# factoryofthesun/distraytracer

Hardware: NVIDIA B200
Metric: samples_per_s_1080p_64spp (higher is better)
Workload: dtype f64

## Files before the change

### distraytracer_b200/csrc/drt_api.cu

```cuda
#include <cuda_runtime.h>

#include <algorithm>
#include <cmath>
#include <cstdio>
#include <cstdlib>
#include <cstring>
#include <string>
#include <vector>

#include "../../include/drt.h"
#include "drt_box.cuh"
#include "drt_launch.h"
#include "drt_bvh_order.h"
#include "drt_mesh.h"
#include "drt_skeleton.h"

using namespace drt;

namespace {

thread_local std::string g_err;
int fail(int code, const std::string& m) { g_err = m; return code; }

#define CK(call)                                                                                   \
// ... 787 lines not shown
int finishRender(drt_scene* s, drt_counters* counters, const Counts& hc, int overflowed) {
  if (overflowed) {
    CK(cudaMemsetAsync(s->overflow, 0, sizeof(int), s->stream));
    CK(cudaStreamSynchronize(s->stream));
    return fail(DRT_ERR_UNSUPPORTED, "a CTA ray pool overflowed (brdf_samples * max_depth beyond the sized bound)");
  }
  if (counters) {
    float ms = 0; CK(cudaEventElapsedTime(&ms, s->ev0, s->ev1));
    counters->kernel_ms = ms;
    if (counters->collect) {
      counters->samples = hc.samples; counters->rays = hc.rays; counters->shadow_rays = hc.shadow_rays;
      counters->shade_evals = hc.shade_evals; counters->noise_evals = hc.noise_evals; counters->node_tests = hc.node_tests;
      for (int i = 0; i < DRT_PRIM_TYPE_COUNT; i++) counters->prim_tests[i] = 0;
      counters->prim_tests[DRT_PRIM_SPHERE] = hc.geom_tests[G_SPHERE];
      counters->prim_tests[DRT_PRIM_CYLINDER] = hc.geom_tests[G_CYL];
      counters->prim_tests[DRT_PRIM_TRIANGLE] = hc.geom_tests[G_TRI];
      counters->prim_tests[DRT_PRIM_RECTANGLE] = hc.geom_tests[G_RECT] + hc.geom_tests[G_CHECKER];
      counters->prim_tests[DRT_PRIM_RECTPRISM] = hc.geom_tests[G_BOX];
    }
  }
  return DRT_OK;
}

int readBack(drt_scene* s, drt_counters* counters, bool check_overflow) {
  Counts hc; memset(&hc, 0, sizeof(hc));
  if (counters && counters->collect) CK(cudaMemcpyAsync(&hc, s->counts, sizeof(Counts), cudaMemcpyDeviceToHost, s->stream));
  int overflowed = 0;
  if (check_overflow) CK(cudaMemcpyAsync(&overflowed, s->overflow, sizeof(int), cudaMemcpyDeviceToHost, s->stream));
  CK(cudaStreamSynchronize(s->stream));
  return finishRender(s, counters, hc, overflowed);
}

int renderCommon(const drt_scene* cs, const drt_settings* st, const drt_tile* tile, float* out_f32, uint8_t* out_u8,
                 drt_counters* counters, bool copy_back) {
  drt_scene* s = const_cast<drt_scene*>(cs);
  int pool_cap = 0;
  CameraD cam;
  int rc = planRender(s, st, tile, pool_cap, cam);
  if (rc) return rc;
  if (tile->device != s->device) return fail(DRT_ERR_INVALID, "tile.device differs from the scene's device");
  CK(cudaSetDevice(s->device));
  const bool want_f32 = out_f32 != nullptr;
  rc = launchFor(s, st, cam, tile, pool_cap, want_f32, counters);
  if (rc) return rc;
  const size_t n_out = (size_t)tile->width * tile->height * 3;
  if (copy_back) {
    if (out_u8) CK(cudaMemcpyAsync(out_u8, s->out_u8, n_out, cudaMemcpyDeviceToHost, s->stream));
    if (out_f32) CK(cudaMemcpyAsync(out_f32, s->out_f32, n_out * sizeof(float), cudaMemcpyDeviceToHost, s->stream));
  }
  return readBack(s, counters, !st->cloud_only);
}

// ... 375 lines not shown
void drt_abi_sizes(int32_t* out6) {
  out6[0] = (int32_t)sizeof(drt_prim); out6[1] = (int32_t)sizeof(drt_light); out6[2] = (int32_t)sizeof(drt_scene_desc);
  out6[3] = (int32_t)sizeof(drt_settings); out6[4] = (int32_t)sizeof(drt_tile); out6[5] = (int32_t)sizeof(drt_counters);
}

int drt_debug_candidate_order(const drt_prim* prims, int32_t n_prims, int32_t* out, int32_t cap) {
  if (!prims || n_prims < 1 || !out) return 0;
  int n = 0;
  for (int i : referenceBVH(prims, n_prims).order) { if (n < cap) out[n] = i; n++; }
  return n;
}

float drt_debug_rng(uint32_t seed, uint32_t pixel, uint32_t sample, uint32_t child, uint32_t dim) {
  uint32_t pk = rng_key_pixel(seed, pixel);
  uint32_t sk = rng_key_sample(pk, sample);
  return rng_u01(rng_key_child(sk, child), dim);
}

int drt_debug_shuffle_j(uint32_t seed, uint32_t pixel, int32_t i) { return rng_shuffle_j(rng_key_pixel(seed, pixel), i); }
int drt_debug_lens_index(uint32_t seed, uint32_t pixel, int32_t sample, int32_t n_lens) {
  return lensIndexScan(rng_key_pixel(seed, pixel), sample, n_lens);
}

}
```

### distraytracer_b200/csrc/drt_device.cuh

```cuda
#pragma once
#include <cuda_runtime.h>
#include <stdint.h>
#include <float.h>
#include <math.h>
#include <utility>

#include "drt_rng.cuh"

#define DRT_PI 3.14159265358979323846
#define DRT_NODE_STACK 64

namespace drt {

template <typename R> struct Vec { R x, y, z; };

template <typename R> __host__ __device__ inline Vec<R> mk(R x, R y, R z) { Vec<R> v; v.x = x; v.y = y; v.z = z; return v; }
template <typename R> __host__ __device__ inline Vec<R> operator+(Vec<R> a, Vec<R> b) { return mk<R>(a.x + b.x, a.y + b.y, a.z + b.z); }
template <typename R> __host__ __device__ inline Vec<R> operator-(Vec<R> a, Vec<R> b) { return mk<R>(a.x - b.x, a.y - b.y, a.z - b.z); }
template <typename R> __host__ __device__ inline Vec<R> operator-(Vec<R> a) { return mk<R>(-a.x, -a.y, -a.z); }
template <typename R> __host__ __device__ inline Vec<R> operator*(Vec<R> a, R s) { return mk<R>(a.x * s, a.y * s, a.z * s); }
template <typename R> __host__ __device__ inline Vec<R> operator*(R s, Vec<R> a) { return mk<R>(s * a.x, s * a.y, s * a.z); }
template <typename R> __host__ __device__ inline Vec<R> operator/(Vec<R> a, R s) { return mk<R>(a.x / s, a.y / s, a.z / s); }
template <typename R> __host__ __device__ inline R dot(Vec<R> a, Vec<R> b) { return a.x * b.x + (a.y * b.y + a.z * b.z); }
template <typename R> __host__ __device__ inline R norm(Vec<R> a) { return sqrt(dot(a, a)); }
// ... 84 lines not shown
  R objM[12];
  Vec<R> center, eA, eB, eC, eD; R e_den;
  Vec<R> vel;
  float height; int n_holes;
  HoleD<R> holes[4];
};

template <typename R>
struct alignas(16) MeshTri {
  Vec<R> A, B, C;
  float uv[6];
};

template <typename R>
struct alignas(16) LightD {
  int type, prim_index;
  float radius;
  int use_baxis;
  float color[3];
  float pad_;
  Vec<R> center, baxis, A, B, D;
};

struct Counts {
  unsigned long long samples, rays, shadow_rays, geom_tests[7], shade_evals, noise_evals, node_tests;
};

template <typename R>
struct Params {
  Vec<R> eye, X, Y, Z;
  R mcam[12], new_mcam[12], cloud_mcam[12];
  float t, b, r, l;
  float near_plane, focal_length, aperture;
  int xRes, yRes;
  int n, spp, antialias_samples;
  int brdf_samples, blur_samples, frame_range, max_depth;
  int reflect, nogloss, perlin_cloud, cloud_only;
  int frame, frame_prism, frame_blur, frame_cloud;
  int swept_cull;
  float move_per_frame, accel_t, refr_air, refr_glass, phong;
  uint32_t seed;
  int blur_mode;
  Vec<R> sun;
  float sun_outer[3], sun_inner[3], sun_core[3], bluesky[3], redsky[3];
  float saturation, clouddist, cloudhoff;
  int x0, y0, w, h;
  const Geom<R>* geoms; int n_geoms;
  const float4* gbounds;
// ... 59 lines not shown
```

### distraytracer_b200/csrc/drt_kernels.cuh

```cuda
#pragma once
#include "drt_device.cuh"
#include "drt_launch.h"
#include <cstddef>

#ifndef DRT_FORCE_TREE
#define DRT_FORCE_TREE 0
#endif

namespace drt {


template <typename R>
struct alignas(16) Task {
  Vec<R> org, dir;
  float k;
  uint32_t path;
  float dt;
  unsigned char depth;
  unsigned char bits;
  unsigned short slot;
};
#define TASK_CHAIN 1
#define TASK_ROOT 2
static_assert(sizeof(Task<double>) == 64 && sizeof(Task<float>) == 48, "ray records are whole 16-byte words");
// ... 329 lines not shown
struct HitRec {
  float t;
  int geom;
  int inside;
  int checker_sel;
};

template <typename R, int F>
__device__ inline bool geomIntersect(const Params<R>& P, const Geom<R>& g, int gi, const int type, const Moved<R>& mv,
                                     const Vec<R>& ray, const Vec<R>& start, float& t_hit, int& inside, int& sel) {
  bool ok = false;
  inside = 0; sel = 0;
    if ((F & FT_BOX) && type == G_BOX) {
      return boxIntersect<R>(P.prims[g.owner], shiftPoint<R, F>(mv, 0, g.vel, g.p0), shiftPoint<R, F>(mv, 0, g.vel, g.p1), ray, start, t_hit, inside, sel);
    } else if (type == G_RECT || type == G_CHECKER) {
      Vec<R> A = shiftPoint<R, F>(mv, g.flags, g.vel, g.p0);
      if (type == G_CHECKER) {
        if (dot(g.p1, ray) == R(0)) return false;
      }
      float c1, c2;
      ok = rectHit<R>(A, g.p1, g.p2, g.p3, g.len1, g.len2, g.eps, ray, start, t_hit, c1, c2);
      if (ok && type == G_CHECKER) {
        if (g.flags & GF_HAS_HOLE) {
          const Geom<R>& hgeo = P.geoms[gi + 1];
          float th, d1, d2;
          if (rectHit<R>(hgeo.p0, hgeo.p1, hgeo.p2, hgeo.p3, hgeo.len1, hgeo.len2, hgeo.eps, ray, start, th, d1, d2))
            ok = false;
        }
        if (ok) {
          int i = (int)(c1 / g.f2);
          int j = (int)(c2 / g.f2);
          int pi = i % 2, pj = j % 2;
          if (pi == 0) { if (pj == 0) sel = 1; if (pj == 1) sel = 2; }
          if (pi == 1) { if (pj == 0) sel = 2; if (pj == 1) sel = 1; }
        }
      }
    } else if (type == G_SPHERE) {
      Vec<R> sc = start - shiftPoint<R, F>(mv, g.flags, g.vel, g.p0);
      float A = (float)dot(ray, ray);
      float B = (float)(R(2) * dot(ray, sc));
      float C = (float)(dot(sc, sc) - (R)((double)g.f0 * (double)g.f0));
      float disc = (float)((double)B * (double)B - (double)(4 * A * C));
      if (disc < 0) return false;
      float sq = sqrtf(disc);
      float t0 = (-B + sq) / (2 * A);
      float t1 = (-B - sq) / (2 * A);
      if (t0 <= 0.001f && t1 <= 0.001f) return false;
// ... 177 lines not shown
    if (ok2 && k2 != kb) stack[sp++] = make_int2(r2, __float_as_int(t2));
    if (ok3 && k3 != kb) stack[sp++] = make_int2(r3, __float_as_int(t3));
    const int bk = kb & 3;
    return bk == 0 ? r0 : bk == 1 ? r1 : bk == 2 ? r2 : r3;
  }
  int nxt = DRT_MESH_DONE;
  if (ok0) nxt = r0;
  if (ok1) { if (nxt != DRT_MESH_DONE) stack[sp++] = make_int2(nxt, 0); nxt = r1; }
  if (ok2) { if (nxt != DRT_MESH_DONE) stack[sp++] = make_int2(nxt, 0); nxt = r2; }
  if (ok3) { if (nxt != DRT_MESH_DONE) stack[sp++] = make_int2(nxt, 0); nxt = r3; }
  return (nxt != DRT_MESH_DONE) ? nxt : bvh4Pop<CLOSEST>(stack, sp, sr.lim);
}

template <typename R, int F, bool COUNT>
__device__ __noinline__ bool gatherReplay(const Params<R>& P, const int leaf, const Vec<R> ray, const Vec<R> start, const Moved<R> mv, Counts& cnt) {
  const Vec<R> inv_ray = mk<R>(R(1) / ray.x, R(1) / ray.y, R(1) / ray.z);
  for (int ni = leaf; ni >= 0; ni = P.nodes[ni].parent) {
    if (COUNT) cnt.node_tests++;
    if (!boxHit<R, F>(P.nodes[ni], ray, inv_ray, start, mv)) return false;
  }
  return true;
}

template <typename R, int F, bool COUNT>
__device__ inline void closestHit(const Params<R>& P, const SlabTab gb, const Moved<R>& mv, const Vec<R>& ray,
                                  const Vec<R>& start, HitRec& h, Counts& cnt) {
  h.t = FLT_MAX; h.geom = -1; h.inside = 0; h.checker_sel = 0;
  if ((!(F & FT_REFBLUR) || mv.val == 0.0f) && !DRT_FORCE_TREE) {
    const float ix = 1.0f / (float)ray.x, iy = 1.0f / (float)ray.y, iz = 1.0f / (float)ray.z;
    const float ox = -(float)start.x * ix, oy = -(float)start.y * iy, oz = -(float)start.z * iz;
    const float serr = 4e-7f * (fabsf(ox) + fabsf(oy) + fabsf(oz));
    const bool cull = !((F & FT_VEL) && mv.velocity_mode) || P.swept_cull;
    const bool smem = !(F & FT_BIG) || P.n_geoms <= DRT_SMEM_GEOMS;
    if ((F & FT_BIG) && cull && P.geom_tree) {
      SlabRay st = slabRay(ix, iy, iz, ox, oy, oz, FLT_MAX);
      int2 stack[DRT_NODE_STACK];
      int sp = 0, cur = 0;
      for (;;) {
        while (cur >= 0) { if (COUNT) cnt.node_tests += 4; cur = bvh4Visit<true>(P.geom_tree, cur, st, stack, sp, P.overflow); }
        if (cur == DRT_MESH_DONE) break;
        const int gi = -cur - 1;
        const Geom<R>& g = P.geoms[gi];
        const int type = g.type;
        if (COUNT) cnt.geom_tests[type]++;
        float t_hit; int inside, sel;
        if (geomIntersect<R, F>(P, g, gi, type, mv, ray, start, t_hit, inside, sel) && (t_hit < h.t || (t_hit == h.t && gi < h.geom)) &&
            (!(F & FT_SPILL) || !(g.flags & GF_SPILL) || ((F & FT_VEL) && mv.velocity_mode) || gatherReplay<R, F, COUNT>(P, g.leaf, ray, start, mv, cnt))) {
          h.t = t_hit; h.geom = gi; h.inside = inside; h.checker_sel = sel;
          st.lim = (t_hit * 1.0001f + 1e-4f) + serr;
        }
        cur = bvh4Pop<true>(stack, sp, st.lim);
      }
      return;
    }
    const SlabRay sr = slabRay(ix, iy, iz, ox, oy, oz, FLT_MAX);
    const int n = P.n_geoms;
    for (int g0 = 0; g0 < n; g0 += 32) {
      const int g1 = min(n, g0 + 32);
      unsigned int mask = !cull ? slabAll(g0, g1) : smem ? slabMask<true>(gb, n, g0, g1, sr) : slabMask<false>(gb, n, g0, g1, sr);
      while (mask) {
        const int gi = g0 + __ffs(mask) - 1;
        mask &= mask - 1;
        const Geom<R>& g = P.geoms[gi];
        const int type = g.type;
        if (type == G_HOLE) continue;
        if (cull && h.t < FLT_MAX && !slabMayHit(g.blo, g.bhi, ox, oy, oz, ix, iy, iz, h.t * 1.0001f + 1e-4f, serr)) continue;
        if (COUNT) cnt.geom_tests[type]++;
        float t_hit; int inside, sel;
        if (geomIntersect<R, F>(P, g, gi, type, mv, ray, start, t_hit, inside, sel) && t_hit < h.t &&
            (!(F & FT_SPILL) || !(g.flags & GF_SPILL) || ((F & FT_VEL) && mv.velocity_mode) || gatherReplay<R, F, COUNT>(P, g.leaf, ray, start, mv, cnt))) {
          h.t = t_hit; h.geom = gi; h.inside = inside; h.checker_sel = sel;
        }
      }
    }
    return;
  }
  int stack[DRT_NODE_STACK];
  int sp = 0;
  stack[sp++] = 0;
  const Vec<R> inv_ray = mk<R>(R(1) / ray.x, R(1) / ray.y, R(1) / ray.z);
  while (sp > 0) {
    const NodeD<R>& nd = P.nodes[stack[--sp]];
    if (COUNT) cnt.node_tests++;
    if (!boxHit<R, F>(nd, ray, inv_ray, start, mv)) continue;
    if (!nd.leaf) { stack[sp++] = nd.left; stack[sp++] = nd.right; continue; }
    const int g_end = nd.first + nd.count;
    for (int gi = nd.first; gi < g_end; gi++) {
      const Geom<R>& g = P.geoms[gi];
      const int type = g.type;
      if (type == G_HOLE) continue;
      if (COUNT) cnt.geom_tests[type]++;
      float t_hit; int inside, sel;
      if (geomIntersect<R, F>(P, g, gi, type, mv, ray, start, t_hit, inside, sel) && t_hit < h.t) {
        h.t = t_hit; h.geom = gi; h.inside = inside; h.checker_sel = sel;
      }
    }
  }
}

template <typename R, int F>
__device__ inline bool geomShadow(const Params<R>& P, const Geom<R>& g, int gi, const int type, const Moved<R>& mv,
                                  const Vec<R>& ray, const Vec<R>& start, const float t_max, float& t_occ, bool& aborted) {
    t_occ = 0.0f;
    if ((F & FT_BOX) && type == G_BOX) {
      return boxShadow<R>(P.prims[g.owner], shiftPoint<R, F>(mv, 0, g.vel, g.p0), shiftPoint<R, F>(mv, 0, g.vel, g.p1), ray, start, t_max, aborted);
    } else if (type == G_RECT || type == G_CHECKER) {
      Vec<R> A = shiftPoint<R, F>(mv, g.flags, g.vel, g.p0);
      float eps = (type == G_CHECKER && !(g.flags & GF_HAS_HOLE)) ? 1e-4f : g.eps;
      float th, c1, c2;
      if (rectHit<R>(A, g.p1, g.p2, g.p3, g.len1, g.len2, eps, ray, start, th, c1, c2) && th < t_max) {
        if (g.flags & GF_HAS_HOLE) {
          const Geom<R>& hgeo = P.geoms[gi + 1];
          float t2, d1, d2;
          if (rectHit<R>(hgeo.p0, hgeo.p1, hgeo.p2, hgeo.p3, hgeo.len1, hgeo.len2, hgeo.eps, ray, start, t2, d1, d2) &&
              t2 < t_max)
            return false;
        }
        t_occ = th;
        return true;
      }
    } else if (type == G_SPHERE) {
      const float eps = 1e-3f;
      Vec<R> sc = start - shiftPoint<R, F>(mv, g.flags, g.vel, g.p0);
      float A = (float)dot(ray, ray);
      float B = (float)(R(2) * dot(ray, sc));
      float C = (float)(dot(sc, sc) - (R)((double)g.f0 * (double)g.f0));
      float disc = (float)((double)B * (double)B - (double)(4 * A * C));
      if (disc < 0) return false;
      float sq = sqrtf(disc);
      float t0 = (-B + sq) / (2 * A);
      float t1 = (-B - sq) / (2 * A);
      if ((t0 <= eps || t0 >= t_max) && (t1 <= eps || t1 >= t_max)) return false;
      t_occ = (t0 > eps && t0 < t_max) ? t0 : t1;
      return true;
    } else if (type == G_CYL) {
// ... 32 lines not shown
      Vec<R> DA0 = cross(A0, r1);
      float v = (float)((double)dot(ray, DA0) * (double)invdet);
      if (v < 0 || u + v > 1) return false;
      float t_final = (float)((double)dot(r2, DA0) * (double)invdet);
      if (t_final > 0.001f && t_final < t_max) { t_occ = t_final; return true; }
    }
  return false;
}

template <typename R, int F, bool COUNT>
__device__ inline bool anyHit(const Params<R>& P, const SlabTab gb, const Moved<R>& mv, const Vec<R>& gather_ray,
                              const Vec<R>& gather_start, const Vec<R>& ray, const Vec<R>& start, float t_max, int skip_owner,
                              Counts& cnt, bool& aborted) {
  if ((!(F & FT_REFBLUR) || mv.val == 0.0f) && !DRT_FORCE_TREE) {
    const float ix = 1.0f / (float)ray.x, iy = 1.0f / (float)ray.y, iz = 1.0f / (float)ray.z;
    const float ox = -(float)start.x * ix, oy = -(float)start.y * iy, oz = -(float)start.z * iz;
    const bool cull = !((F & FT_VEL) && mv.velocity_mode) || P.swept_cull;
    const float gather_lead = t_max * 1e-3f;
    const int n = P.n_geoms;
    const bool smem = !(F & FT_BIG) || n <= DRT_SMEM_GEOMS;
    const SlabRay sr = slabRay(ix, iy, iz, ox, oy, oz, t_max * 1.0001f + 1e-4f);
    auto candidate = [&](const int gi) -> int {
      const Geom<R>& g = P.geoms[gi];
      const int type = g.type;
      if (type == G_HOLE || g.owner == skip_owner) return 0;
      if (COUNT) cnt.geom_tests[type]++;
      float t_occ;
      if (!geomShadow<R, F>(P, g, gi, type, mv, ray, start, t_max, t_occ, aborted)) return ((F & FT_BOX) && aborted) ? -1 : 0;
      if ((F & FT_VEL) && mv.velocity_mode) return 1;
      if (t_occ > gather_lead * 1.001f + 2e-3f && !((F & FT_SPILL) && (g.flags & GF_SPILL))) return 1;
      return gatherReplay<R, F, COUNT>(P, g.leaf, gather_ray, gather_start, mv, cnt) ? 1 : 0;
    };
    if ((F & FT_BIG) && cull && P.geom_tree) {
      int2 stack[DRT_NODE_STACK];
      int sp = 0, cur = 0;
      for (;;) {
        while (cur >= 0) { if (COUNT) cnt.node_tests += 4; cur = bvh4Visit<false>(P.geom_tree, cur, sr, stack, sp, P.overflow); }
        if (cur == DRT_MESH_DONE) break;
        if (candidate(-cur - 1) == 1) return true;
        cur = bvh4Pop<false>(stack, sp, sr.lim);
      }
      return false;
    }
    for (int g0 = 0; g0 < n; g0 += 32) {
      const int g1 = min(n, g0 + 32);
      unsigned int mask = !cull ? slabAll(g0, g1) : smem ? slabMask<true>(gb, n, g0, g1, sr) : slabMask<false>(gb, n, g0, g1, sr);
      while (mask) {
// ... 189 lines not shown
    double spec;
    if (phong == 10.0f) { const double b2 = base * base, b4 = b2 * b2; spec = b4 * b4 * b2; }
    else spec = drt_pow(base, (double)phong);
    for (int c = 0; c < 3; c++) {
      double sh = (double)Lcolor[c] * lam + (double)Lcolor[c] * spec;
      ray_color[c] = (double)shape_color[c] * sh;
    }
  }
}

struct alignas(16) HitRef {
  float t;
  int geom;
  int inside_sel;
  int slot;
};

template <typename R>
__device__ __forceinline__ int meshOwner(const Params<R>& P, const int tri) {
  return P.mesh_prim + (P.mesh_mat ? (int)__ldg(P.mesh_mat + tri) : 0);
}

template <typename R, int F, bool COUNT>
__device__ inline bool traceRay(const Params<R>& P, const SlabTab gb, const Task<R>& T, HitRec& h, int& motion,
                                Counts& cnt) {
  motion = -1;
  if (T.depth == 0) return false;
  if (COUNT) cnt.rays++;
  const Moved<R> mv = makeMoved<R, F>(P, T.dt);
  closestHit<R, F, COUNT>(P, gb, mv, T.dir, T.org, h, cnt);
  if ((F & FT_MESH) && P.n_mesh_tris > 0) {
    meshTraverse<R, F, COUNT, true>(P, T.dir, T.org, h.t, &h, T.dir, T.org, (F & FT_VEL) && mv.velocity_mode, mv.time, cnt);
  }
  if ((F & (FT_VEL | FT_REFBLUR)) && (T.bits & TASK_CHAIN)) motion = 0;
  if (h.geom < 0) return false;
  if ((F & (FT_VEL | FT_REFBLUR)) && (T.bits & TASK_CHAIN)) {
    const int owner = h.geom >= P.n_geoms ? meshOwner(P, h.geom - P.n_geoms) : P.geoms[h.geom].owner;
    motion = (P.prims[owner].flags & 2) ? 1 : 0;
  }
  return true;
}

template <typename R>
struct ShadeState {
  Vec<R> isectP, normal, e;
  Moved<R> mv;
  float shape_color[3];
  float k;
  uint32_t path;
  int prim;
  int tri;
  bool lights;
  bool aborted, early;
  int hits;
  double tmp[3];
};

template <typename R>
struct PairIn {
  Vec<R> isectP;
  uint32_t path;
  float val, dt;
  int want;
};
template <typename R>
struct PairOut {
  R* x; R* y; R* z;
  unsigned char* state;
};
template <typename R>
__host__ __device__ constexpr size_t pairOutBytes() { return (size_t)32 * DRT_PAIR_LIGHTS * 3 * sizeof(R); }

template <typename R, int F, bool COUNT>
__device__ void shadeA(const Params<R>& P, const Task<R>& T, const HitRec& h, Task<R>* stack, int& n_out, double (&add)[3],
                       bool& has_add, bool& aborted, ShadeState<R>& S, Counts& cnt) {
  int sp = 0;
  n_out = 0; has_add = false;
  add[0] = add[1] = add[2] = 0.0;
  const Moved<R> mv = makeMoved<R, F>(P, T.dt);
  S.lights = false; S.aborted = false; S.early = false; S.hits = 0; S.tmp[0] = S.tmp[1] = S.tmp[2] = 0.0; S.mv = mv;
  do {
    const Vec<R> ray = T.dir, eye = T.org;
    const float k = T.k;
    const int mesh_tri = ((F & FT_MESH) && h.geom >= P.n_geoms) ? h.geom - P.n_geoms : -1;
    const int owner = mesh_tri >= 0 ? meshOwner(P, mesh_tri) : P.geoms[h.geom].owner;
    const PrimD<R>& pr = P.prims[owner];

    const Vec<R> isectP = eye + (R)h.t * ray;
    Vec<R> normal;
    if (pr.type == 0) {
      Vec<R> nn = isectP - shiftPoint<R, F>(mv, 0, pr.vel, pr.pA);
      normal = nn / norm(nn);
    } else if (pr.type == 1 || pr.type == 7) {
      const Vec<R> c1 = shiftPoint<R, F>(mv, 0, pr.vel, pr.pA);
      Vec<R> axis = pr.pG;
      if ((F & FT_VEL) && (pr.flags & 64) && mv.velocity_mode) axis = normalized((pr.n1 + pr.n2 * mv.time) - c1);
      Vec<R> pc = isectP - c1;
      normal = normalized(pc - dot(pc, axis) * axis);
    } else if ((F & FT_BOX) && pr.type == 9) {
      const float eps = 1e-3f;
      const Vec<R> pa = isectP - shiftPoint<R, F>(mv, 0, pr.vel, pr.pA);
      if (dot(pa, pr.n0) <= (R)eps) normal = pr.n0;
      else if (dot(pa, pr.n1) <= (R)eps) normal = pr.n1;
      else if (dot(pa, pr.n2) <= (R)eps) normal = pr.n2;
      else { aborted = true; break; }
    } else if ((F & FT_BOX) && pr.type == 10) {
      normal = prismHolesNorm<R>(pr, isectP, h.checker_sel >= 3 ? h.checker_sel - 3 : -1, aborted);
      if (aborted) break;
// ... 351 lines not shown
    float r = (float)((double)(P.aperture / 2) * (double)rng_u01(pkey, 4u * li));
    float theta = (float)(2 * DRT_PI * (double)rng_u01(pkey, 4u * li + 1));
    double snd, csd;
    sincos((double)theta, &snd, &csd);
    const float cs = (float)csd, sn = (float)snd;
    eye_sample = P.eye + (R)(r * cs) * P.X + (R)(r * sn) * P.Y;
  }
  const int ii = s / P.n, jj = s % P.n;
  float adj_x = (float)((double)x + ((double)(float)ii + (double)rng_u01(pkey, 4u * s + 2)) / 9.0);
  float adj_y = (float)((double)y + ((double)(float)jj + (double)rng_u01(pkey, 4u * s + 3)) / 9.0);
  pi = (int)(double)adj_x; pj = (int)(double)adj_y;
  const Vec<R> rayDir = eyeRay<R>(P, pi, pj);
  const Vec<R> focalPoint = P.eye + (R)P.focal_length * rayDir;
  org = eye_sample;
  dir = focalPoint - eye_sample;
}

#ifndef DRT_WAVE_CTAS_PER_SM
#define DRT_WAVE_CTAS_PER_SM 1
#endif
#define DRT_HIT_BUCKETS 64
__host__ __device__ constexpr size_t waveDynSmemBytes() { return (size_t)DRT_CTA_SLOTS * 28 + (size_t)DRT_CTA_HITS * 3; }
template <typename R>
__host__ __device__ constexpr size_t waveScratchBytes(int pool_cap) {
  return (size_t)pool_cap * sizeof(Task<R>) + DRT_CTA_HITS * sizeof(HitRef) + DRT_WAVE_WARPS * pairOutBytes<R>() +
         3 * (size_t)(pool_cap / 32) * sizeof(uint32_t);
}

template <typename R, int F, bool COUNT>
__global__ void __launch_bounds__(32 * DRT_WAVE_WARPS, DRT_WAVE_CTAS_PER_SM) render_wave(const __grid_constant__ Params<R> P) {
  extern __shared__ __align__(16) unsigned char s_dyn[];
  unsigned long long(*s_acc)[3] = (unsigned long long(*)[3])s_dyn;
  unsigned int* s_flags = (unsigned int*)(s_dyn + (size_t)DRT_CTA_SLOTS * 24);
  unsigned short* s_order = (unsigned short*)(s_dyn + (size_t)DRT_CTA_SLOTS * 28);
  unsigned char* s_hkey = s_dyn + (size_t)DRT_CTA_SLOTS * 28 + (size_t)DRT_CTA_HITS * 2;
  __shared__ int s_nst, s_nfree, s_ninfl, s_npush, s_count, s_nhits, s_grab, s_state, s_nvalid;
  __shared__ int s_hist[DRT_HIT_BUCKETS];
  __shared__ long long s_idx0, s_unit_next, s_unit_end;
  __shared__ float4 s_gb[3 * DRT_SMEM_GEOMS / 2 + 2 * DRT_SMEM_GEOMS / 8];
  SlabTab gb; gb.g = P.gbounds; gb.s = 0u;
  if (!(F & FT_BIG) || P.n_geoms <= DRT_SMEM_GEOMS) {
    for (int i = threadIdx.x; i < slabPairWords(P.n_geoms) + 2 * ((P.n_geoms + 7) / 8); i += blockDim.x) s_gb[i] = P.gbounds[i];
    gb.s = (unsigned)__cvta_generic_to_shared(s_gb);
  }
  const unsigned FULL = 0xffffffffu;
  const int lane = threadIdx.x & 31, wib = threadIdx.x >> 5, tid = threadIdx.x;
  const size_t cap = (size_t)P.pool_cap;
  const int n_chunks = P.pool_cap >> 5;
  char* cbase = (char*)P.pool_raw + (size_t)blockIdx.x * waveScratchBytes<R>(P.pool_cap);
  uint4* pool = (uint4*)cbase;
  uint4* hits = (uint4*)(cbase + cap * sizeof(Task<R>));
  char* wbase = (char*)(hits + DRT_CTA_HITS) + (size_t)wib * pairOutBytes<R>();
  uint32_t* stk = (uint32_t*)((char*)(hits + DRT_CTA_HITS) + (size_t)DRT_WAVE_WARPS * pairOutBytes<R>());
  uint32_t* fre = stk + n_chunks;
  uint32_t* infl = fre + n_chunks;
  PairOut<R> pairout;
  __shared__ unsigned char s_pstate[DRT_WAVE_WARPS * 32 * DRT_PAIR_LIGHTS];
  pairout.x = (R*)wbase; pairout.y = pairout.x + 32 * DRT_PAIR_LIGHTS; pairout.z = pairout.y + 32 * DRT_PAIR_LIGHTS;
  pairout.state = s_pstate + wib * 32 * DRT_PAIR_LIGHTS;
  unsigned long long(*acc)[3] = s_acc;
  unsigned int* sfl = s_flags;
  const long long n_units = (P.sample_count + P.unit_samples - 1) / P.unit_samples;

  Counts cnt;
  if (COUNT) { cnt.samples = 0; cnt.rays = 0; cnt.shadow_rays = 0; cnt.shade_evals = 0; cnt.noise_evals = 0; cnt.node_tests = 0;
               for (int i = 0; i < 7; i++) cnt.geom_tests[i] = 0; }

  for (int i = tid; i < n_chunks; i += blockDim.x) __stcg(fre + i, (uint32_t)(n_chunks - 1 - i));
  if (tid == 0) { s_nst = 0; s_nfree = n_chunks; s_ninfl = 0; s_npush = 0; s_count = 0; s_nhits = 0; s_state = 0; s_nvalid = 0;
                  s_idx0 = 0; s_unit_next = 0; s_unit_end = 0; }
  __syncthreads();

  for (;;) {
    if (s_nst == 0 && s_nhits == 0) {
      const int state = s_state;
      const int n_valid = s_nvalid;
      const long long idx0 = s_idx0;
      const int f0 = s_nfree;
      __syncthreads();
      bool finalize = false;
      if ((F & (FT_VEL | FT_REFBLUR)) && state == 1 && P.blur_samples > 0) {
        int mine = 0;
        for (int s2 = tid; s2 < n_valid; s2 += blockDim.x) mine |= ((sfl[s2] & (SS_MOTION | SF_ABORT)) == SS_MOTION);
        if (__syncthreads_or(mine)) {
          const bool have_perm = lensSwapTargetsFill<R>(P, P.sample_base + idx0, n_valid, s_order, DRT_CTA_HITS);
          const int perm_pt0 = (int)((P.sample_base + idx0) / P.spp);
          for (int s2 = tid; s2 < n_valid; s2 += blockDim.x) {
            if ((sfl[s2] & (SS_MOTION | SF_ABORT)) != SS_MOTION) continue;
            Task<R> T; uint32_t skey; int pi, pj, px, py;
// ... 69 lines not shown
        __syncthreads();
        if (s_state == 3) break;
        const int nv = s_nvalid;
        const long long i0 = s_idx0;
        for (int s2 = tid; s2 < DRT_CTA_SLOTS; s2 += blockDim.x) { acc[s2][0] = acc[s2][1] = acc[s2][2] = 0ull; sfl[s2] = 0u; }
        const bool have_perm = lensSwapTargetsFill<R>(P, P.sample_base + i0, nv, s_order, DRT_CTA_HITS);
        const int perm_pt0 = (int)((P.sample_base + i0) / P.spp);
        const int nch = (nv + 31) >> 5;
        for (int s2 = tid; s2 < nch * 32; s2 += blockDim.x) {
          const uint32_t id = __ldcg(fre + f0 - 1 - (s2 >> 5));
          if ((s2 & 31) == 0) __stcg(stk + (s2 >> 5), id);
          if (s2 >= nv) { poolStoreEmpty<Task<R>>(pool, cap, (int)id * 32 + (s2 & 31)); continue; }
          Task<R> T; uint32_t skey; int pi, pj, px, py;
          primaryRay<R>(P, P.sample_base + i0 + s2, have_perm ? s_order : nullptr, perm_pt0, true, T.org, T.dir, skey, pi, pj, px, py);
          T.k = 1.0f; T.path = rng_key_child(skey, 0); T.dt = 0.f; T.depth = (unsigned char)P.max_depth;
          T.bits = TASK_CHAIN | TASK_ROOT; T.slot = (unsigned short)s2;
          poolStore(pool, cap, (int)id * 32 + (s2 & 31), T);
          if (COUNT) cnt.samples++;
        }
        if (tid == 0) { s_nst = nch; s_nfree = f0 - nch; }
      }
      __syncthreads();
    }

    const int nst0 = s_nst;
    if (tid == 0) { s_grab = nst0; s_count = 0; }
    __syncthreads();
    for (;;) {
      if (((volatile int*)&s_nhits)[0] >= DRT_TRACE_HITS_TARGET) break;
      int top = 0;
      uint32_t id = 0;
      if (lane == 0) { top = atomicSub(&s_grab, 1); if (top > 0) id = __ldcg(stk + top - 1); }
      top = __shfl_sync(FULL, top, 0);
      if (top <= 0) break;
      id = __shfl_sync(FULL, id, 0);
      const int slot = (int)id * 32 + lane;
      bool hit = false;
      HitRec h; h.t = 0.f; h.geom = -1; h.inside = 0; h.checker_sel = 0;
      {
        Task<R> T;
        poolLoad<Task<R>, true>(T, pool, cap, slot);
        if (T.depth != 0 && !(((volatile unsigned int*)sfl)[T.slot] & SF_ABORT)) {
          int motion;
          hit = traceRay<R, F, COUNT>(P, gb, T, h, motion, cnt);
          unsigned int orf = 0;
          if ((T.bits & TASK_ROOT) && hit) orf |= SS_HIT;
          if (motion == 1) orf |= SS_MOTION;
          if (orf) atomicOr(&sfl[T.slot], orf);
          if (motion == 0) atomicAnd(&sfl[T.slot], ~SS_MOTION);
        }
      }
      const unsigned int hm = __ballot_sync(FULL, hit);
      int hbase = 0;
      if (lane == 0) {
        if (hm) { hbase = atomicAdd(&s_nhits, __popc(hm)); __stcg(infl + atomicAdd(&s_ninfl, 1), id); }
        else __stcg(fre + atomicAdd(&s_nfree, 1), id);
      }
      hbase = __shfl_sync(FULL, hbase, 0);
      if (hit) {
        const int at = hbase + __popc(hm & ((1u << lane) - 1u));
        __stcg(hits + at, make_uint4(__float_as_uint(h.t), (unsigned)h.geom, (unsigned)(h.inside | (h.checker_sel << 1)), (unsigned)slot));
        s_hkey[at] = (unsigned char)min(h.geom, DRT_HIT_BUCKETS - 1);
      }
    }
    __syncthreads();
    const int nh = s_nhits;
    const int nst_base = max(s_grab, 0);
    __syncthreads();
    if (tid == 0) s_grab = nh;
    for (int i = tid; i < DRT_HIT_BUCKETS; i += blockDim.x) s_hist[i] = 0;
    __syncthreads();
    int rank[(DRT_CTA_HITS + 32 * DRT_WAVE_WARPS - 1) / (32 * DRT_WAVE_WARPS)];
#pragma unroll
    for (int k = 0; k < (DRT_CTA_HITS + 32 * DRT_WAVE_WARPS - 1) / (32 * DRT_WAVE_WARPS); k++) {
      const int i = tid + k * 32 * DRT_WAVE_WARPS;
      rank[k] = (i < nh) ? atomicAdd(&s_hist[s_hkey[i]], 1) : 0;
    }
    __syncthreads();
    if (wib == 0) {
      int run = 0;
      for (int b0 = 0; b0 < DRT_HIT_BUCKETS; b0 += 32) {
        const int c = s_hist[b0 + lane];
        int incl = c;
#pragma unroll
        for (int d = 1; d < 32; d <<= 1) { int v = __shfl_up_sync(FULL, incl, d); if (lane >= d) incl += v; }
        s_hist[b0 + lane] = run + incl - c;
        run += __shfl_sync(FULL, incl, 31);
      }
    }
    __syncthreads();
#pragma unroll
    for (int k = 0; k < (DRT_CTA_HITS + 32 * DRT_WAVE_WARPS - 1) / (32 * DRT_WAVE_WARPS); k++) {
      const int i = tid + k * 32 * DRT_WAVE_WARPS;
      if (i < nh) s_order[s_hist[s_hkey[i]] + rank[k]] = (unsigned short)i;
    }
    __syncthreads();

    int open_id = -1, open_fill = 0;
    for (;;) {
      int end = 0;
      if (lane == 0) end = atomicSub(&s_grab, 32);
      end = __shfl_sync(FULL, end, 0);
      if (end <= 0) break;
      const int begin = max(end - 32, 0);
      const int take = end - begin;
      const bool active = lane < take;
      Task<R> kids[DRT_MAX_CHILDREN];
      int nk = 0;
      ShadeState<R> S; S.lights = false; S.aborted = false;
      double add[3] = {0, 0, 0}; bool has_add = false, aborted = false;
      unsigned short slot = 0;
      PairIn<R> pin; pin.want = 0; pin.isectP = mk<R>(R(0), R(0), R(0)); pin.path = 0u; pin.val = 0.f; pin.dt = 0.f;
      if (active) {
        const uint4 hr = __ldcs(hits + (int)s_order[end - 1 - lane]);
        Task<R> T;
        poolLoad<Task<R>, true>(T, pool, cap, (int)hr.w);
        HitRec h; h.t = __uint_as_float(hr.x); h.geom = (int)hr.y; h.inside = (int)(hr.z & 1u); h.checker_sel = (int)(hr.z >> 1);
        slot = T.slot;
        shadeA<R, F, COUNT>(P, T, h, kids, nk, add, has_add, aborted, S, cnt);
        if (!aborted && S.lights) { pin.isectP = S.isectP; pin.path = T.path; pin.val = S.mv.val; pin.dt = T.dt; pin.want = 1; }
      }
      for (int l0 = 0; l0 < P.n_lights; l0 += DRT_PAIR_LIGHTS) {
        const int nl = min(DRT_PAIR_LIGHTS, P.n_lights - l0);
        for (int p0 = 0; p0 < take * nl; p0 += 32) {
          const int pid = p0 + lane;
          const bool on = pid < take * nl;
          const int lj = on ? pid / take : 0, hh = on ? pid - lj * take : 0;
          PairIn<R> q;
          q.isectP = mk<R>(__shfl_sync(FULL, pin.isectP.x, hh), __shfl_sync(FULL, pin.isectP.y, hh), __shfl_sync(FULL, pin.isectP.z, hh));
          q.path = __shfl_sync(FULL, pin.path, hh);
          q.val = (F & FT_REFBLUR) ? __shfl_sync(FULL, pin.val, hh) : 0.f;
          q.dt = (F & (FT_VEL | FT_REFBLUR)) ? __shfl_sync(FULL, pin.dt, hh) : 0.f;
          q.want = __shfl_sync(FULL, pin.want, hh);
          if (on && q.want) shadowPair<R, F, COUNT>(P, gb, q, l0 + lj, pairout, lj * 32 + hh, cnt);
        }
        __syncwarp();
        if (active && !aborted && S.lights) shadeB<R, F, COUNT>(P, S, pairout, lane, l0, l0 + nl, cnt);
        __syncwarp();
      }
      if (active) {
        if (S.lights && !aborted) {
          if (S.aborted) aborted = true;
          else if (!S.early && S.hits > 0) { for (int c = 0; c < 3; c++) add[c] += S.tmp[c] / S.hits; has_add = true; }
        }
        if (aborted) { atomicOr(&sfl[slot], SF_ABORT); nk = 0; }
        else if (has_add) {
          unsigned int orf = 0;
          for (int c = 0; c < 3; c++) {
            const double v = add[c];
            if (v != v) orf |= SS_NAN(c);
            else if (v > 1073741824.0) orf |= SS_PINF(c);
            else if (v < -1073741824.0) orf |= SS_NINF(c);
            else atomicAdd(&acc[slot][c], (unsigned long long)__double2ll_rn(v * 4294967296.0));
          }
          if (orf) atomicOr(&sfl[slot], orf);
        }
      }
      const int total = __reduce_add_sync(FULL, nk);
      if (total) {
        const int have = open_id >= 0 ? 1 : 0;
        const int touched = (open_fill + total + 31) >> 5;
// ... 20 lines not shown
          const int full = base >> 5;
          int pp = 0;
          if (lane == 0 && full) pp = atomicAdd(&s_npush, full);
          pp = __shfl_sync(FULL, pp, 0);
          if (lane < full) __stcg(stk + nst_base + pp + lane, (uint32_t)myid);
          open_fill = base & 31;
          open_id = __shfl_sync(FULL, myid, min(full, 31));
          if (!open_fill) open_id = -1;
        }
      }
    }
    if (open_id >= 0) {
      if (lane >= open_fill) poolStoreEmpty<Task<R>>(pool, cap, open_id * 32 + lane);
      if (lane == 0) __stcg(stk + nst_base + atomicAdd(&s_npush, 1), (uint32_t)open_id);
    }
    __syncthreads();
    {
      const int ninfl = s_ninfl, f = s_nfree;
      for (int i = tid; i < ninfl; i += blockDim.x) __stcg(fre + f + i, __ldcg(infl + i));
      __syncthreads();
      if (tid == 0) { s_nfree = f + ninfl; s_ninfl = 0; s_nst = nst_base + s_npush; s_npush = 0; s_nhits = 0; }
    }
    __syncthreads();
  }

  if (COUNT) {
    atomicAdd(&P.counts->samples, cnt.samples); atomicAdd(&P.counts->rays, cnt.rays);
    atomicAdd(&P.counts->shadow_rays, cnt.shadow_rays); atomicAdd(&P.counts->shade_evals, cnt.shade_evals);
    atomicAdd(&P.counts->node_tests, cnt.node_tests);
    for (int i = 0; i < 7; i++) if (cnt.geom_tests[i]) atomicAdd(&P.counts->geom_tests[i], cnt.geom_tests[i]);
  }
}

__constant__ int kNoisePrimes[10][3] = {{995615039, 600173719, 701464987}, {831731269, 162318869, 136250887},
                                        {174329291, 946737083, 245679977}, {362489573, 795918041, 350777237},
                                        {457025711, 880830799, 909678923}, {787070341, 177340217, 593320781},
                                        {405493717, 291031019, 391950901}, {458904767, 676625681, 424452397},
                                        {531736441, 939683957, 810651871}, {997169939, 842027887, 423882827}};

__device__ __forceinline__ float noiseLattice(const uint32_t a, const uint32_t b, const uint32_t c, const int n) {
  uint32_t un = (uint32_t)n;
  un = (un << 13) ^ un;
  const int t = (int)((un * (un * un * a + b) + c) & 0x7fffffffu);
  const double td = __hiloint2double(0x43300000, t) - 4503599627370496.0;
  return (float)(1.0 - td * (1.0 / 1073741823.0));
}
__device__ __forceinline__ double latticeWiden(const float f) {
  const uint32_t u = __float_as_uint(f);
  const uint32_t hi = (u & 0x80000000u) | (((u >> 3) & 0x0fffffffu) + 0x38000000u);
  return __hiloint2double((int)hi, (int)(u << 29));
}
__device__ inline double cosInterp(double a, double b, double x) {
  double f = (1 - cos(x * DRT_PI)) * 0.5;
// ... 187 lines not shown
```

### distraytracer_b200/csrc/drt_launch_impl.cuh

```cuda
#include <algorithm>
#include "drt_kernels.cuh"
#include "drt_launch.h"

namespace drt {
typedef WaveFnT<DRT_REAL> WaveFn;
#define DRT_WAVE_CASE(mask) if (feat == (mask) && !collect) return render_wave<DRT_REAL, (mask), false>
#if DRT_GROUP == 0
template <> WaveFn waveKernelOfGroup<DRT_REAL, 0>(int feat, bool collect) {
  DRT_WAVE_CASE(FT_GLASS | FT_TEX);
  DRT_WAVE_CASE(0);
  DRT_WAVE_CASE(FT_TEX);
  return nullptr;
}
#elif DRT_GROUP == 1
template <> WaveFn waveKernelOfGroup<DRT_REAL, 1>(int feat, bool collect) {
  DRT_WAVE_CASE(FT_VEL);
  DRT_WAVE_CASE(FT_MESH | FT_TEX);
  DRT_WAVE_CASE(FT_MESH | FT_VEL | FT_TEX);
  return nullptr;
}
#else
template <> WaveFn waveKernelOfGroup<DRT_REAL, 2>(int feat, bool collect) {
  DRT_WAVE_CASE(FT_REFBLUR | FT_GLASS | FT_TEX);
  DRT_WAVE_CASE(FT_ALL);
  if (feat == FT_ALL && collect) return render_wave<DRT_REAL, FT_ALL, true>;
  return nullptr;
}
#endif

#if DRT_GROUP == 0
static WaveFn waveKernel(int feat, bool collect) {
  WaveFn f = waveKernelOfGroup<DRT_REAL, 0>(feat, collect);
  if (!f) f = waveKernelOfGroup<DRT_REAL, 1>(feat, collect);
  if (!f) f = waveKernelOfGroup<DRT_REAL, 2>(feat, collect);
  return f;
}
template <> int waveGridBlocks<DRT_REAL>() {
  int dev = 0, sms = 0, per_sm = 1 << 30, n = 0;
  cudaGetDevice(&dev);
  cudaDeviceGetAttribute(&sms, cudaDevAttrMultiProcessorCount, dev);
  const int* list = waveFeatList(&n);
  for (int i = 0; i <= n; i++) {
    WaveFn f = i < n ? waveKernel(list[i], false) : waveKernel(FT_ALL, true);
    int k = 0;
    cudaFuncSetAttribute((const void*)f, cudaFuncAttributeMaxDynamicSharedMemorySize, (int)waveDynSmemBytes());
    cudaOccupancyMaxActiveBlocksPerMultiprocessor(&k, (const void*)f, 32 * DRT_WAVE_WARPS, waveDynSmemBytes());
    per_sm = k < per_sm ? k : per_sm;
  }
  if (per_sm < 1) per_sm = 1;
  return sms * per_sm;
}
template <> size_t wavePoolBytes<DRT_REAL>(int blocks, int pool_cap) { return (size_t)blocks * waveScratchBytes<DRT_REAL>(pool_cap); }
template <> int launchRenderSamples<DRT_REAL>(const Params<DRT_REAL>& P, bool collect, int feat, int blocks, cudaStream_t q) {
  const int pick = collect ? FT_ALL : waveFeatPick(feat);
  waveKernel(pick, collect)<<<blocks, 32 * DRT_WAVE_WARPS, waveDynSmemBytes(), q>>>(P);
  return pick;
}
template <> void launchCloudCorners<DRT_REAL>(const Params<DRT_REAL>& P, cudaStream_t q) {
  const int n = (P.w + 1) * (P.h + 1);
  int blocks = (n + DRT_CLOUD_BLOCK - 1) / DRT_CLOUD_BLOCK;
  if (P.corner_counter) {
    int dev = 0, sms = 0;
    cudaGetDevice(&dev);
    cudaDeviceGetAttribute(&sms, cudaDevAttrMultiProcessorCount, dev);
    blocks = std::min(blocks, sms * 16);
  }
  cloud_corners<DRT_REAL><<<blocks, 128, 0, q>>>(P);
}
#ifdef DRT_DEFINE_SHARED_LAUNCHERS
void launchNeedPush(const unsigned char* mine, unsigned char* shared, size_t n, cudaStream_t q) {
  need_push<<<(unsigned)((n + 255) / 256), 256, 0, q>>>(mine, shared, n);
}
#endif
template <> void launchResolve<DRT_REAL>(const Params<DRT_REAL>& P, int row0, int rows, cudaStream_t q) {
  resolve<DRT_REAL><<<(P.w * rows + 255) / 256, 256, 0, q>>>(P, row0, rows);
}
#endif
}
// ... 1 lines not shown
```

Before: 775.1.

## Stage geometry records into shared memory for non-BIG wave kernels

For scenes without the FT_BIG feature, each CTA copies the whole Geom array into dynamic shared memory at kernel start. closestHit, traceRay and shadeA then read from that copy through a new pointer parameter instead of from global memory. Hole lookups now use the neighbouring record of the current geom. The occupancy calculation and the launch now include the extra shared bytes, which can lower blocks per SM. Optional phase-clock instrumentation, compiled out by default, is added for profiling.

```diff
diff --git a/distraytracer_b200/csrc/drt_api.cu b/distraytracer_b200/csrc/drt_api.cu
--- a/distraytracer_b200/csrc/drt_api.cu
+++ b/distraytracer_b200/csrc/drt_api.cu
@@ -833,12 +833,19 @@
   return DRT_OK;
 }
 
+#if DRT_PHASE_CLOCKS
+static unsigned long long g_phase_clocks[PC_COUNT];
+#endif
+
 int readBack(drt_scene* s, drt_counters* counters, bool check_overflow) {
   Counts hc; memset(&hc, 0, sizeof(hc));
   if (counters && counters->collect) CK(cudaMemcpyAsync(&hc, s->counts, sizeof(Counts), cudaMemcpyDeviceToHost, s->stream));
   int overflowed = 0;
   if (check_overflow) CK(cudaMemcpyAsync(&overflowed, s->overflow, sizeof(int), cudaMemcpyDeviceToHost, s->stream));
   CK(cudaStreamSynchronize(s->stream));
+#if DRT_PHASE_CLOCKS
+  if (counters && counters->collect) memcpy(g_phase_clocks, hc.clk, sizeof(g_phase_clocks));
+#endif
   return finishRender(s, counters, hc, overflowed);
 }
 
@@ -1260,4 +1267,10 @@
   return lensIndexScan(rng_key_pixel(seed, pixel), sample, n_lens);
 }
 
-}
+#if DRT_PHASE_CLOCKS
+int drt_debug_phase_clocks(uint64_t* out, int32_t cap) {
+  for (int i = 0; i < PC_COUNT && i < cap; i++) out[i] = g_phase_clocks[i];
+  return PC_COUNT;
+}
+#endif
+}
diff --git a/distraytracer_b200/csrc/drt_device.cuh b/distraytracer_b200/csrc/drt_device.cuh
--- a/distraytracer_b200/csrc/drt_device.cuh
+++ b/distraytracer_b200/csrc/drt_device.cuh
@@ -130,8 +130,16 @@
   Vec<R> center, baxis, A, B, D;
 };
 
+#ifndef DRT_PHASE_CLOCKS
+#define DRT_PHASE_CLOCKS 0
+#endif
+enum PhaseClock { PC_GEN, PC_TRACE, PC_SORT, PC_SHADE_A, PC_STEP_B, PC_STEP_C, PC_BOOK, PC_GEOM_WAIT, PC_GEOM_LOADS, PC_COUNT };
+
 struct Counts {
   unsigned long long samples, rays, shadow_rays, geom_tests[7], shade_evals, noise_evals, node_tests;
+#if DRT_PHASE_CLOCKS
+  unsigned long long clk[PC_COUNT];
+#endif
 };
 
 template <typename R>
diff --git a/distraytracer_b200/csrc/drt_kernels.cuh b/distraytracer_b200/csrc/drt_kernels.cuh
--- a/distraytracer_b200/csrc/drt_kernels.cuh
+++ b/distraytracer_b200/csrc/drt_kernels.cuh
@@ -375,7 +375,7 @@
       ok = rectHit<R>(A, g.p1, g.p2, g.p3, g.len1, g.len2, g.eps, ray, start, t_hit, c1, c2);
       if (ok && type == G_CHECKER) {
         if (g.flags & GF_HAS_HOLE) {
-          const Geom<R>& hgeo = P.geoms[gi + 1];
+          const Geom<R>& hgeo = (&g)[1];
           float th, d1, d2;
           if (rectHit<R>(hgeo.p0, hgeo.p1, hgeo.p2, hgeo.p3, hgeo.len1, hgeo.len2, hgeo.eps, ray, start, th, d1, d2))
             ok = false;
@@ -599,8 +599,25 @@
   return true;
 }
 
+template <bool COUNT, typename R>
+__device__ __forceinline__ int candidateType(const Geom<R>& g, Counts& cnt) {
+#if DRT_PHASE_CLOCKS
+  if (COUNT) {
+    const long long t0 = clock64();
+    asm volatile("" ::: "memory");
+    const int type = g.type;
+    int one;
+    asm volatile("{ .reg .pred p; setp.ge.s32 p, %1, 0; selp.s32 %0, 1, 0, p; }" : "=r"(one) : "r"(type));
+    const long long t1 = clock64();
+    if ((__activemask() & ((1u << (threadIdx.x & 31)) - 1u)) == 0) { cnt.clk[PC_GEOM_WAIT] += t1 - t0; cnt.clk[PC_GEOM_LOADS] += one; }
+    return type;
+  }
+#endif
+  return g.type;
+}
+
 template <typename R, int F, bool COUNT>
-__device__ inline void closestHit(const Params<R>& P, const SlabTab gb, const Moved<R>& mv, const Vec<R>& ray,
+__device__ inline void closestHit(const Params<R>& P, const SlabTab gb, const Geom<R>* geoms, const Moved<R>& mv, const Vec<R>& ray,
                                   const Vec<R>& start, HitRec& h, Counts& cnt) {
   h.t = FLT_MAX; h.geom = -1; h.inside = 0; h.checker_sel = 0;
   if ((!(F & FT_REFBLUR) || mv.val == 0.0f) && !DRT_FORCE_TREE) {
@@ -617,7 +634,7 @@
         while (cur >= 0) { if (COUNT) cnt.node_tests += 4; cur = bvh4Visit<true>(P.geom_tree, cur, st, stack, sp, P.overflow); }
         if (cur == DRT_MESH_DONE) break;
         const int gi = -cur - 1;
-        const Geom<R>& g = P.geoms[gi];
+        const Geom<R>& g = geoms[gi];
         const int type = g.type;
         if (COUNT) cnt.geom_tests[type]++;
         float t_hit; int inside, sel;
@@ -638,8 +655,8 @@
       while (mask) {
         const int gi = g0 + __ffs(mask) - 1;
         mask &= mask - 1;
-        const Geom<R>& g = P.geoms[gi];
-        const int type = g.type;
+        const Geom<R>& g = geoms[gi];
+        const int type = candidateType<COUNT>(g, cnt);
         if (type == G_HOLE) continue;
         if (cull && h.t < FLT_MAX && !slabMayHit(g.blo, g.bhi, ox, oy, oz, ix, iy, iz, h.t * 1.0001f + 1e-4f, serr)) continue;
         if (COUNT) cnt.geom_tests[type]++;
@@ -663,7 +680,7 @@
     if (!nd.leaf) { stack[sp++] = nd.left; stack[sp++] = nd.right; continue; }
     const int g_end = nd.first + nd.count;
     for (int gi = nd.first; gi < g_end; gi++) {
-      const Geom<R>& g = P.geoms[gi];
+      const Geom<R>& g = geoms[gi];
       const int type = g.type;
       if (type == G_HOLE) continue;
       if (COUNT) cnt.geom_tests[type]++;
@@ -687,7 +704,7 @@
       float th, c1, c2;
       if (rectHit<R>(A, g.p1, g.p2, g.p3, g.len1, g.len2, eps, ray, start, th, c1, c2) && th < t_max) {
         if (g.flags & GF_HAS_HOLE) {
-          const Geom<R>& hgeo = P.geoms[gi + 1];
+          const Geom<R>& hgeo = (&g)[1];
           float t2, d1, d2;
           if (rectHit<R>(hgeo.p0, hgeo.p1, hgeo.p2, hgeo.p3, hgeo.len1, hgeo.len2, hgeo.eps, ray, start, t2, d1, d2) &&
               t2 < t_max)
@@ -766,7 +783,7 @@
     const SlabRay sr = slabRay(ix, iy, iz, ox, oy, oz, t_max * 1.0001f + 1e-4f);
     auto candidate = [&](const int gi) -> int {
       const Geom<R>& g = P.geoms[gi];
-      const int type = g.type;
+      const int type = candidateType<COUNT>(g, cnt);
       if (type == G_HOLE || g.owner == skip_owner) return 0;
       if (COUNT) cnt.geom_tests[type]++;
       float t_occ;
@@ -1002,20 +1019,20 @@
 }
 
 template <typename R, int F, bool COUNT>
-__device__ inline bool traceRay(const Params<R>& P, const SlabTab gb, const Task<R>& T, HitRec& h, int& motion,
+__device__ inline bool traceRay(const Params<R>& P, const SlabTab gb, const Geom<R>* geoms, const Task<R>& T, HitRec& h, int& motion,
                                 Counts& cnt) {
   motion = -1;
   if (T.depth == 0) return false;
   if (COUNT) cnt.rays++;
   const Moved<R> mv = makeMoved<R, F>(P, T.dt);
-  closestHit<R, F, COUNT>(P, gb, mv, T.dir, T.org, h, cnt);
+  closestHit<R, F, COUNT>(P, gb, geoms, mv, T.dir, T.org, h, cnt);
   if ((F & FT_MESH) && P.n_mesh_tris > 0) {
     meshTraverse<R, F, COUNT, true>(P, T.dir, T.org, h.t, &h, T.dir, T.org, (F & FT_VEL) && mv.velocity_mode, mv.time, cnt);
   }
   if ((F & (FT_VEL | FT_REFBLUR)) && (T.bits & TASK_CHAIN)) motion = 0;
   if (h.geom < 0) return false;
   if ((F & (FT_VEL | FT_REFBLUR)) && (T.bits & TASK_CHAIN)) {
-    const int owner = h.geom >= P.n_geoms ? meshOwner(P, h.geom - P.n_geoms) : P.geoms[h.geom].owner;
+    const int owner = h.geom >= P.n_geoms ? meshOwner(P, h.geom - P.n_geoms) : geoms[h.geom].owner;
     motion = (P.prims[owner].flags & 2) ? 1 : 0;
   }
   return true;
@@ -1052,7 +1069,7 @@
 __host__ __device__ constexpr size_t pairOutBytes() { return (size_t)32 * DRT_PAIR_LIGHTS * 3 * sizeof(R); }
 
 template <typename R, int F, bool COUNT>
-__device__ void shadeA(const Params<R>& P, const Task<R>& T, const HitRec& h, Task<R>* stack, int& n_out, double (&add)[3],
+__device__ void shadeA(const Params<R>& P, const Geom<R>* geoms, const Task<R>& T, const HitRec& h, Task<R>* stack, int& n_out, double (&add)[3],
                        bool& has_add, bool& aborted, ShadeState<R>& S, Counts& cnt) {
   int sp = 0;
   n_out = 0; has_add = false;
@@ -1063,7 +1080,7 @@
     const Vec<R> ray = T.dir, eye = T.org;
     const float k = T.k;
     const int mesh_tri = ((F & FT_MESH) && h.geom >= P.n_geoms) ? h.geom - P.n_geoms : -1;
-    const int owner = mesh_tri >= 0 ? meshOwner(P, mesh_tri) : P.geoms[h.geom].owner;
+    const int owner = mesh_tri >= 0 ? meshOwner(P, mesh_tri) : geoms[h.geom].owner;
     const PrimD<R>& pr = P.prims[owner];
 
     const Vec<R> isectP = eye + (R)h.t * ray;
@@ -1461,6 +1478,11 @@
 #define DRT_HIT_BUCKETS 64
 __host__ __device__ constexpr size_t waveDynSmemBytes() { return (size_t)DRT_CTA_SLOTS * 28 + (size_t)DRT_CTA_HITS * 3; }
 template <typename R>
+__host__ __device__ constexpr size_t waveGeomSmemBytes(int feat, int n_geoms) {
+  return (feat & FT_BIG) ? 0 : (size_t)n_geoms * sizeof(Geom<R>);
+}
+static_assert(DRT_CTA_SLOTS * 28 % 16 == 0 && DRT_CTA_HITS * 3 % 16 == 0, "the staged Geom records start 16-byte aligned");
+template <typename R>
 __host__ __device__ constexpr size_t waveScratchBytes(int pool_cap) {
   return (size_t)pool_cap * sizeof(Task<R>) + DRT_CTA_HITS * sizeof(HitRef) + DRT_WAVE_WARPS * pairOutBytes<R>() +
          3 * (size_t)(pool_cap / 32) * sizeof(uint32_t);
@@ -1481,6 +1503,12 @@
   if (!(F & FT_BIG) || P.n_geoms <= DRT_SMEM_GEOMS) {
     for (int i = threadIdx.x; i < slabPairWords(P.n_geoms) + 2 * ((P.n_geoms + 7) / 8); i += blockDim.x) s_gb[i] = P.gbounds[i];
     gb.s = (unsigned)__cvta_generic_to_shared(s_gb);
+  }
+  const Geom<R>* geoms = P.geoms;
+  if (!(F & FT_BIG)) {
+    uint4* s_geoms = (uint4*)(s_dyn + waveDynSmemBytes());
+    for (int i = threadIdx.x; i < P.n_geoms * (int)(sizeof(Geom<R>) / 16); i += blockDim.x) s_geoms[i] = __ldg((const uint4*)P.geoms + i);
+    geoms = (const Geom<R>*)s_geoms;
   }
   const unsigned FULL = 0xffffffffu;
   const int lane = threadIdx.x & 31, wib = threadIdx.x >> 5, tid = threadIdx.x;
@@ -1504,6 +1532,13 @@
   Counts cnt;
   if (COUNT) { cnt.samples = 0; cnt.rays = 0; cnt.shadow_rays = 0; cnt.shade_evals = 0; cnt.noise_evals = 0; cnt.node_tests = 0;
                for (int i = 0; i < 7; i++) cnt.geom_tests[i] = 0; }
+#if DRT_PHASE_CLOCKS
+  if (COUNT) for (int i = 0; i < PC_COUNT; i++) cnt.clk[i] = 0;
+  long long clk0 = clock64();
+#define DRT_PHASE(k) do { if (COUNT) { __syncwarp(); const long long t_ = clock64(); cnt.clk[k] += t_ - clk0; clk0 = t_; } } while (0)
+#else
+#define DRT_PHASE(k) do { } while (0)
+#endif
 
   for (int i = tid; i < n_chunks; i += blockDim.x) __stcg(fre + i, (uint32_t)(n_chunks - 1 - i));
   if (tid == 0) { s_nst = 0; s_nfree = n_chunks; s_ninfl = 0; s_npush = 0; s_count = 0; s_nhits = 0; s_state = 0; s_nvalid = 0;
@@ -1619,6 +1654,7 @@
       }
       __syncthreads();
     }
+    DRT_PHASE(PC_GEN);
 
     const int nst0 = s_nst;
     if (tid == 0) { s_grab = nst0; s_count = 0; }
@@ -1639,7 +1675,7 @@
         poolLoad<Task<R>, true>(T, pool, cap, slot);
         if (T.depth != 0 && !(((volatile unsigned int*)sfl)[T.slot] & SF_ABORT)) {
           int motion;
-          hit = traceRay<R, F, COUNT>(P, gb, T, h, motion, cnt);
+          hit = traceRay<R, F, COUNT>(P, gb, geoms, T, h, motion, cnt);
           unsigned int orf = 0;
           if ((T.bits & TASK_ROOT) && hit) orf |= SS_HIT;
           if (motion == 1) orf |= SS_MOTION;
@@ -1661,6 +1697,7 @@
       }
     }
     __syncthreads();
+    DRT_PHASE(PC_TRACE);
     const int nh = s_nhits;
     const int nst_base = max(s_grab, 0);
     __syncthreads();
@@ -1692,6 +1729,7 @@
       if (i < nh) s_order[s_hist[s_hkey[i]] + rank[k]] = (unsigned short)i;
     }
     __syncthreads();
+    DRT_PHASE(PC_SORT);
 
     int open_id = -1, open_fill = 0;
     for (;;) {
@@ -1714,9 +1752,10 @@
         poolLoad<Task<R>, true>(T, pool, cap, (int)hr.w);
         HitRec h; h.t = __uint_as_float(hr.x); h.geom = (int)hr.y; h.inside = (int)(hr.z & 1u); h.checker_sel = (int)(hr.z >> 1);
         slot = T.slot;
-        shadeA<R, F, COUNT>(P, T, h, kids, nk, add, has_add, aborted, S, cnt);
+        shadeA<R, F, COUNT>(P, geoms, T, h, kids, nk, add, has_add, aborted, S, cnt);
         if (!aborted && S.lights) { pin.isectP = S.isectP; pin.path = T.path; pin.val = S.mv.val; pin.dt = T.dt; pin.want = 1; }
       }
+      DRT_PHASE(PC_SHADE_A);
       for (int l0 = 0; l0 < P.n_lights; l0 += DRT_PAIR_LIGHTS) {
         const int nl = min(DRT_PAIR_LIGHTS, P.n_lights - l0);
         for (int p0 = 0; p0 < take * nl; p0 += 32) {
@@ -1732,8 +1771,10 @@
           if (on && q.want) shadowPair<R, F, COUNT>(P, gb, q, l0 + lj, pairout, lj * 32 + hh, cnt);
         }
         __syncwarp();
+        DRT_PHASE(PC_STEP_B);
         if (active && !aborted && S.lights) shadeB<R, F, COUNT>(P, S, pairout, lane, l0, l0 + nl, cnt);
         __syncwarp();
+        DRT_PHASE(PC_STEP_C);
       }
       if (active) {
         if (S.lights && !aborted) {
@@ -1800,13 +1841,19 @@
       if (tid == 0) { s_nfree = f + ninfl; s_ninfl = 0; s_nst = nst_base + s_npush; s_npush = 0; s_nhits = 0; }
     }
     __syncthreads();
-  }
+    DRT_PHASE(PC_BOOK);
+  }
+#undef DRT_PHASE
 
   if (COUNT) {
     atomicAdd(&P.counts->samples, cnt.samples); atomicAdd(&P.counts->rays, cnt.rays);
     atomicAdd(&P.counts->shadow_rays, cnt.shadow_rays); atomicAdd(&P.counts->shade_evals, cnt.shade_evals);
     atomicAdd(&P.counts->node_tests, cnt.node_tests);
     for (int i = 0; i < 7; i++) if (cnt.geom_tests[i]) atomicAdd(&P.counts->geom_tests[i], cnt.geom_tests[i]);
+#if DRT_PHASE_CLOCKS
+    for (int i = 0; i < PC_COUNT; i++)
+      if ((lane == 0 || i >= PC_GEOM_WAIT) && cnt.clk[i]) atomicAdd(&P.counts->clk[i], cnt.clk[i]);
+#endif
   }
 }
 
diff --git a/distraytracer_b200/csrc/drt_launch_impl.cuh b/distraytracer_b200/csrc/drt_launch_impl.cuh
--- a/distraytracer_b200/csrc/drt_launch_impl.cuh
+++ b/distraytracer_b200/csrc/drt_launch_impl.cuh
@@ -10,6 +10,9 @@
   DRT_WAVE_CASE(FT_GLASS | FT_TEX);
   DRT_WAVE_CASE(0);
   DRT_WAVE_CASE(FT_TEX);
+#if DRT_PHASE_CLOCKS
+  if (feat == (FT_GLASS | FT_TEX) && collect) return render_wave<DRT_REAL, FT_GLASS | FT_TEX, true>;
+#endif
   return nullptr;
 }
 #elif DRT_GROUP == 1
@@ -43,17 +46,25 @@
   for (int i = 0; i <= n; i++) {
     WaveFn f = i < n ? waveKernel(list[i], false) : waveKernel(FT_ALL, true);
     int k = 0;
-    cudaFuncSetAttribute((const void*)f, cudaFuncAttributeMaxDynamicSharedMemorySize, (int)waveDynSmemBytes());
-    cudaOccupancyMaxActiveBlocksPerMultiprocessor(&k, (const void*)f, 32 * DRT_WAVE_WARPS, waveDynSmemBytes());
+    const int feat = i < n ? list[i] : FT_ALL;
+    const size_t dyn = waveDynSmemBytes() + waveGeomSmemBytes<DRT_REAL>(feat, DRT_SMEM_GEOMS);
+    cudaFuncSetAttribute((const void*)f, cudaFuncAttributeMaxDynamicSharedMemorySize, (int)dyn);
+    cudaOccupancyMaxActiveBlocksPerMultiprocessor(&k, (const void*)f, 32 * DRT_WAVE_WARPS, dyn);
     per_sm = k < per_sm ? k : per_sm;
   }
+#if DRT_PHASE_CLOCKS
+  cudaFuncSetAttribute((const void*)waveKernel(FT_GLASS | FT_TEX, true), cudaFuncAttributeMaxDynamicSharedMemorySize,
+                       (int)(waveDynSmemBytes() + waveGeomSmemBytes<DRT_REAL>(FT_GLASS | FT_TEX, DRT_SMEM_GEOMS)));
+#endif
   if (per_sm < 1) per_sm = 1;
   return sms * per_sm;
 }
 template <> size_t wavePoolBytes<DRT_REAL>(int blocks, int pool_cap) { return (size_t)blocks * waveScratchBytes<DRT_REAL>(pool_cap); }
 template <> int launchRenderSamples<DRT_REAL>(const Params<DRT_REAL>& P, bool collect, int feat, int blocks, cudaStream_t q) {
-  const int pick = collect ? FT_ALL : waveFeatPick(feat);
-  waveKernel(pick, collect)<<<blocks, 32 * DRT_WAVE_WARPS, waveDynSmemBytes(), q>>>(P);
+  int pick = waveFeatPick(feat);
+  if (collect && !(DRT_PHASE_CLOCKS && pick == (FT_GLASS | FT_TEX))) pick = FT_ALL;
+  const size_t dyn = waveDynSmemBytes() + waveGeomSmemBytes<DRT_REAL>(pick, P.n_geoms);
+  waveKernel(pick, collect)<<<blocks, 32 * DRT_WAVE_WARPS, dyn, q>>>(P);
   return pick;
 }
 template <> void launchCloudCorners<DRT_REAL>(const Params<DRT_REAL>& P, cudaStream_t q) {
```

Result: no change. 781.3, median of 6 (+0.8%).
